# lan496/torch-m3gnet

Measured on AMD Instinct MI355X. Metric: atom-steps/sec (energy+forces) on 10k-atom PBC batch, 1/2/4/8 MI355X, higher is better.
Workload: dtype f32; 1 GPU; single 10000-atom fcc Cu PBC supercell per GPU (10x10x25 cells, a=3.61 A, jitter 0.025 A), r_cut 5 A / 3-body 4 A, default M3GNet (l_max=n_max=3, D=64, 3 blocks), energy+forces+stress; precision=fp32, atoms_per_gpu=10000, edges_per_gpu=420000, triplets_per_gpu=3060000

## Files before the change

### torch-m3gnet_amd/csrc/m3g_api.hip

```cpp
#include <climits>
#include <cmath>
#include <cstdarg>
#include <cstdio>
#include <cstdlib>
#include <cstring>
#include <utility>

#include "m3g_internal.h"

namespace m3g {

static thread_local char g_err[512] = "";
void set_error(const char* fmt, ...) {
  va_list ap;
  va_start(ap, fmt);
  vsnprintf(g_err, sizeof(g_err), fmt, ap);
  va_end(ap);
}

static void layout_mlp(MlpW& m, size_t& off) {
  auto take = [&](size_t n) { size_t r = off; off += (n + 63) / 64 * 64; return r; };
  m.w1a_t = take(kDP * 2 * kDP); m.w1b_t = take(kDP * 2 * kDP); m.w1c_t = take(kDP * 2 * kDP);
  m.b1 = take(2 * kDP);
  m.w2d_t = take(kDP * kDP); m.w2g_t = take(kDP * kDP);
// ... 277 lines not shown
  auto it = exp.find(key);
  if (it == exp.end()) { set_error("unknown parameter key '%s'", key); return M3G_ERR_VALUE; }
  if (it->second != numel) { set_error("parameter '%s': expected %lld values, got %lld", key, (long long)it->second, (long long)numel); return M3G_ERR_VALUE; }
  plan->params[key].assign(host_data, host_data + numel);
  plan->committed = false;
  return M3G_OK;
}

extern "C" int m3g_plan_set_const(m3g_plan* plan, const char* name, const float* host_data, int64_t numel) {
  if (!plan || !name || !host_data) { set_error("m3g_plan_set_const: null argument"); return M3G_ERR_VALUE; }
  auto exp = expected_consts(plan->cfg);
  auto it = exp.find(name);
  if (it == exp.end()) { set_error("unknown constant '%s'", name); return M3G_ERR_VALUE; }
  if (it->second != numel) { set_error("constant '%s': expected %lld values, got %lld", name, (long long)it->second, (long long)numel); return M3G_ERR_VALUE; }
  plan->cvals[name].assign(host_data, host_data + numel);
  plan->committed = false;
  return M3G_OK;
}

static int hook_stamps(m3g_plan* plan, int32_t* value) {
  if (*value && !plan->d_stamps) {
    M3G_HIP_CHECK(hipMalloc((void**)&plan->d_stamps, 256 * 16 * 12 * sizeof(unsigned long long)));
    M3G_HIP_CHECK(hipMemset(plan->d_stamps, 0, 256 * 16 * 12 * sizeof(unsigned long long)));
  } else if (!*value && plan->d_stamps) {
    (void)hipFree(plan->d_stamps);
    plan->d_stamps = nullptr;
  }
  *value = *value == 0 ? 0 : *value == 3 ? 3 : *value == 2 ? 2 : 1;
  return M3G_OK;
}
struct OptionRow {
  const char* name;
  int Options::*member;
  int lo, hi;
  const char* error;
  int (*hook)(m3g_plan*, int32_t* value);
};
#define M3G_HOOK(...) [](m3g_plan* plan, int32_t* value) -> int { __VA_ARGS__; return M3G_OK; }
static const OptionRow kOptions[] = {
    {"edge_kernel", &Options::edge_kernel, 0, 2, "edge_kernel must be 0 (VALU baseline), 1 (MFMA) or 2 (any-size path)",
     M3G_HOOK(if (plan->generic && *value != 2) { set_error("this model size only runs on the any-size path (edge_kernel = 2)"); return M3G_ERR_UNSUPPORTED; })},
    {"precision", &Options::precision, 0, 2,
     "precision must be 0 (fp32: exact fp32 MFMA products), 1 (bf16x3 split products) or 2 (f16x3: scaled fp16 split products)", nullptr},
    {"save_p1", &Options::save_p1, 0, 1, nullptr, nullptr},
    {"save_p2", &Options::save_p2, 0, 1, nullptr, nullptr},
    {"rev_kernel", &Options::rev_kernel, 0, 1, "rev_kernel must be 0 (node-MLP + edge-MLP kernel pair) or 1 (fused)", nullptr},
    {"small_tiles", &Options::small_tiles, 0, INT_MAX, "small_tiles must be >= 0", M3G_HOOK(plan->opt.small_tiles_fwd = *value)},
    {"small_tiles_fwd", &Options::small_tiles_fwd, 0, INT_MAX, "small_tiles_fwd must be >= 0", nullptr},
    {"dp1_by_dst", &Options::dp1_by_dst, 0, 1, nullptr, nullptr},
    {"split_node_tiles", &Options::split_node_tiles, 0, INT_MAX, "split_node_tiles must be >= 0", nullptr},
    {"species_tables", &Options::species_tables, 0, 1, nullptr, nullptr},
    {"fuse_node_tb", &Options::fuse_node_tb, 0, 1, nullptr, nullptr},
    {"debug_node_tb_polls", &Options::debug_node_tb_polls, INT_MIN, INT_MAX, nullptr, nullptr},
    {"split_tail", &Options::split_tail, 0, 2, "split_tail must be 0 (never), 1 (a single left-over tile) or 2 (one or two)", nullptr},
    {"small_launches", &Options::small_launches, 0, 1, nullptr, nullptr},
    {"graph_replay", &Options::graph_replay, 0, 1, nullptr, M3G_HOOK(if (!*value) drop_graphs(plan))},
    {"overlap", &Options::overlap, 0, 1, nullptr, nullptr},
    {"threebody_moments", &Options::tb_moments, 0, 1, nullptr, nullptr},
    {"legendre_backward", &Options::legendre_ref, 0, 1, "legendre_backward: 0 (exact derivative) or 1 (the reference's backward)", nullptr},
    {"readout_f16", &Options::readout_f16, 0, 1, nullptr, nullptr},
    {"stress_mode", &Options::stress_mode, 0, 1, "stress_mode must be 0 (reference: sum pos (x) F / V) or 1 (pair virial)", nullptr},
    {"debug_force_move", nullptr, INT_MIN, INT_MAX, nullptr, M3G_HOOK(plan->debug_force_move = *value != 0; plan->committed = false)},
    {"stamps", &Options::stamp_target, INT_MIN, INT_MAX, nullptr, hook_stamps},
};
#undef M3G_HOOK

extern "C" int m3g_plan_set_option(m3g_plan* plan, const char* name, int32_t value) {
  if (!plan || !name) { set_error("m3g_plan_set_option: null argument"); return M3G_ERR_VALUE; }
  for (const OptionRow& row : kOptions) {
    if (strcmp(name, row.name) != 0) continue;
    if (value < row.lo || value > row.hi) {
      if (row.error) { set_error("%s", row.error); return M3G_ERR_VALUE; }
      value = 1;
    }
    if (row.hook) { int rc = row.hook(plan, &value); if (rc) return rc; }
    if (row.member) plan->opt.*row.member = value;
    return M3G_OK;
  }
  set_error("unknown option '%s'", name);
  return M3G_ERR_VALUE;
}

extern "C" int m3g_debug_read_stamps(m3g_plan* plan, uint64_t* host_out ) {
  if (!plan || !host_out || !plan->d_stamps) { set_error("stamps not enabled"); return M3G_ERR_STATE; }
  M3G_HIP_CHECK(hipMemcpy(host_out, plan->d_stamps, 256 * 16 * 12 * sizeof(unsigned long long), hipMemcpyDeviceToHost));
  return M3G_OK;
}

extern "C" int m3g_plan_commit(m3g_plan* plan) {
  if (!plan) { set_error("m3g_plan_commit: null plan"); return M3G_ERR_VALUE; }
  drop_graphs(plan);
  const m3g_config& cfg = plan->cfg;
  for (auto& kv : expected_params(cfg))
    if (!plan->params.count(kv.first)) { set_error("parameter '%s' was never set", kv.first.c_str()); return M3G_ERR_STATE; }
  for (auto& kv : expected_consts(cfg))
    if (!plan->cvals.count(kv.first)) { set_error("constant '%s' was never set", kv.first.c_str()); return M3G_ERR_STATE; }
  const int D = cfg.embedding_dim, R = cfg.n_max, L = cfg.l_max, C = L * R, B = cfg.num_blocks;
  {
    int dev = 0;
    M3G_HIP_CHECK(hipGetDevice(&dev));
    if (plan->device >= 0 && (plan->device != dev || plan->debug_force_move)) {
      M3G_HIP_CHECK(hipSetDevice(plan->device));
      M3G_HIP_CHECK(hipDeviceSynchronize());
      if (plan->d_weights) { (void)hipFree(plan->d_weights); plan->d_weights = nullptr; }
      free_mfma_images(plan);
      generic_free(plan);
// ... 176 lines not shown

int Step::enqueue_optional_outputs() const {
  M3G_STAGE(ST_OUTPUTS);
  if (io->node_features) launch_copy_strided(w.x[c.B], kDP, io->node_features, c.D, c.D, t.N, s);
  if (io->edge_attr) {
    if (mfma) launch_soa_to_rows(w.e_blk[c.B], io->edge_attr, c.D, c.D, t.E, s);
    else launch_copy_strided(w.e, kDP, io->edge_attr, c.D, c.D, t.E, s);
  }
  if (io->edge_distances && t.E > 0) M3G_HIP_CHECK(hipMemcpyAsync(io->edge_distances, w.d, sizeof(float) * t.E, hipMemcpyDeviceToDevice, s));
  if (io->edge_weights) launch_copy_strided(w.h, kRP, io->edge_weights, c.R, c.R, t.E, s);
  if (io->triplet_angles) launch_triplet_angles(t, io->triplet_edge_index, w.u, io->triplet_angles, s);
  if (io->mid_edge_features)
    for (int b = 0; b < c.B; ++b)
      launch_copy_expand_rows(t.act_id, w.m[b], kCP, io->mid_edge_features + (size_t)b * t.E * c.C, c.C, c.C, t.E, s);
  return M3G_OK;
}

int Step::enqueue_reverse() const {
  float *dx_cur = w.dx, *dx_alt = w.dx2;
  bool dr_done = false;
  if (!mfma && c.B > 0 && t.E > 0) {
    M3G_HIP_CHECK(hipMemsetAsync(w.de, 0, sizeof(float) * t.E * kDP, s));
    M3G_HIP_CHECK(hipMemsetAsync(w.dh, 0, sizeof(float) * t.E * kRP, s));
  }
  for (int b = c.B - 1; b >= 0; --b) {
    const bool first = b == c.B - 1;
    switch (p.rev_edge) {
      case kRevSplit: { M3G_STAGE(ST_EDGE_REV_FUSED); launch_edge_rev_split(plan, p, c, t, w, b, dx_cur, first, s); } break;
      case kRevF32: { M3G_STAGE(ST_EDGE_REV_FUSED); launch_edge_rev_f32(plan, p, c, t, w, b, dx_cur, first, s); } break;
      case kRevFused: { M3G_STAGE(ST_EDGE_REV_FUSED); launch_edge_rev_fused(plan, c, t, w, b, dx_cur, first, s); } break;
      case kRevPair: {
        { M3G_STAGE(ST_EDGE_REV_NODE); launch_edge_rev_node_mlp(plan, p, c, t, w, b, dx_cur, s); }
        M3G_STAGE(ST_EDGE_REV);
        launch_edge_rev_edge_mlp(plan, p, c, t, w, b, dx_cur, first, s);
      } break;
      default: { M3G_STAGE(ST_EDGE_REV); launch_edge_block_reverse(c, W, wl.blk[b], t, w, b, dx_cur, s); }
    }
    bool node_done = false;
    if (p.tail[b] == kTailOverlap) {
      if (!ensure_side_stream(plan)) { set_error("overlap: could not create the internal stream"); return M3G_ERR_HIP; }
      M3G_HIP_CHECK(hipEventRecord(plan->ev_fork, s));
      M3G_HIP_CHECK(hipStreamWaitEvent(plan->side_stream, plan->ev_fork, 0));
      launch_threebody_reverse(p, c, t, w, w.v[b], first, plan->side_stream, plan->opt.legendre_ref);
      M3G_HIP_CHECK(hipEventRecord(plan->ev_join, plan->side_stream));
      launch_node_reverse(c, W, wl.blk[b], t, w, w.v[b], dx_cur, dx_alt, true, p.dp1, false, s);
      M3G_HIP_CHECK(hipStreamWaitEvent(s, plan->ev_join, 0));
      launch_node_reverse_v_term(c, W, wl.blk[b], t, w, w.v[b], dx_alt, s);
      node_done = true;
    } else if (p.tail[b] == kTailNodeTb) {
      node_done = launch_node_tb_reverse(c, W, wl.blk[b], t, w, w.v[b], first, dx_cur, dx_alt, p.dp1, b, s, p.tb_hints, plan->opt.debug_node_tb_polls);
    } else if (p.tail[b] == kTailFinalTb) {
      launch_threebody_reverse_final(c, t, w, w.v[b], first, w.dh_parts, c.B, s, p.tb_hints);
      dr_done = true;
    }
    if (!node_done && p.tail[b] != kTailFinalTb) {
      { M3G_STAGE(ST_THREEBODY_REV); launch_threebody_reverse(p, c, t, w, w.v[b], first, s, plan->opt.legendre_ref); }
      if (b > 0) {
        M3G_STAGE(ST_NODE_REV);
        launch_node_reverse(c, W, wl.blk[b], t, w, w.v[b], dx_cur, dx_alt, p.fused_rev, p.dp1, true, s, p.node_rev_small);
        node_done = true;
      }
    }
    if (node_done) std::swap(dx_cur, dx_alt);
  }
  {
    M3G_STAGE(ST_EMBED_REV);
    if (p.fused_rev) {  }
    else if (mfma) launch_embed_edges_reverse_soa(W + wl.adj, w.h, w.de_soa, w.dh_parts + (size_t)2 * c.B * t.E * kRP, t.E, s);
    else launch_embed_reverse(c, W, wl, t, w, s);
  }
  M3G_STAGE(ST_GEOM_REV);
  if (mfma) launch_geometry_reverse(c, t, w, w.dh_parts, p.fused_rev ? c.B : 2 * c.B + 1, io->forces, io->stresses, s, p.gather_virial, io->pos, io->lattice, dr_done);
  else launch_geometry_reverse(c, t, w, w.dh, 1, io->forces, io->stresses, s);
  if (p.stress == kStressPair) launch_stress_pair(t, w, io->lattice, io->stresses, s);
  else if (p.stress == kStressRef) launch_stress(c, t, io->pos, io->lattice, io->forces, io->stresses, s, p.energy_deferred ? ea : nullptr, st, io->total_energy);
  return M3G_OK;
}

static int enqueue_step(const m3g_plan* plan, const m3g_io* io, void* workspace, size_t workspace_bytes, hipStream_t s, RunMode mode) {
  const int64_t N = io->n_atoms, E = io->n_edges, T = io->n_triplets, S = io->n_structs;
  if (N < 0 || E < 0 || T < 0 || S < 0) { set_error("negative size"); return M3G_ERR_VALUE; }
  if (!io->total_energy || !io->topo || (N > 0 && (!io->pos || !io->atom_types)) || (S > 0 && !io->lattice) || (E > 0 && !io->edge_cell_shift)) {
    set_error("m3g_energy_forces: missing required pointer");
    return M3G_ERR_VALUE;
  }
  if (io->triplet_angles && T > 0 && !io->triplet_edge_index) { set_error("triplet_angles requires triplet_edge_index"); return M3G_ERR_VALUE; }
  const StepPath p = plan_step_path(plan, N, E, T, S, io->topo_hints, io->forces != nullptr, io->stresses != nullptr, mode.profile);
  if (p.pipeline == kPipeAnySize) return generic_energy_forces(plan, io, workspace, workspace_bytes, s);
  Step k{plan, io, p, p.pipeline == kPipeMfma, plan->consts, plan->wl, plan->d_weights, s, mode, topo_carve(N, E, T, S, const_cast<void*>(io->topo)),
         work_carve(plan->cfg.num_blocks, p, N, E, S, workspace)};
  if (!workspace || workspace_bytes < k.w.total_bytes) { set_error("workspace too small: %zu < %zu", workspace_bytes, k.w.total_bytes); return M3G_ERR_SIZE; }
  k.ea = io->scaled_atomic_energies ? io->scaled_atomic_energies : k.w.tail;
  k.st = io->scaled_total_energy ? io->scaled_total_energy : k.w.tail + N;
  { int rc = k.enqueue_forward(); if (rc) return rc; }
  { int rc = k.enqueue_optional_outputs(); if (rc) return rc; }
  if (io->forces) { int rc = k.enqueue_reverse(); if (rc) return rc; }
  else if (io->stresses) { set_error("stresses require forces"); return M3G_ERR_VALUE; }
  M3G_HIP_CHECK(hipGetLastError());
  return M3G_OK;
}

static int capture_step(const m3g_plan* plan, const m3g_io* io, void* workspace, size_t workspace_bytes, hipStream_t s, hipGraph_t* graph) {
  M3G_HIP_CHECK(hipStreamBeginCapture(s, hipStreamCaptureModeThreadLocal));
  const int rc = enqueue_step(plan, io, workspace, workspace_bytes, s, RunMode{false});
  const hipError_t e = hipStreamEndCapture(s, graph);
  if (rc != M3G_OK) { if (*graph) (void)hipGraphDestroy(*graph); return rc; }
// ... 127 lines not shown
```

### torch-m3gnet_amd/csrc/m3g_internal.h

```cpp
#pragma once
#include <hip/hip_runtime.h>

#include <cmath>
#include <cstddef>
#include <cstdint>
#include <map>
#include <string>
#include <vector>

#include "../../include/m3gnet_hip.h"
#include "m3g_step_path.h"

namespace m3g {

constexpr int kDP = 64;
constexpr int kLCap = 4;
constexpr int kRCap = 4;
constexpr int kRAnyCap = 10;
constexpr int kCP = 16;
constexpr int kRP = 4;

void set_error(const char* fmt, ...);
#define M3G_HIP_CHECK(expr)                                                               \
  do {                                                                                    \
// ... 319 lines not shown
void launch_stress(const Consts& c, const Topo& t, const float* pos, const float* lattice, const float* forces,
                   float* stresses, hipStream_t s, const float* ea = nullptr, float* scaled_total = nullptr, float* total = nullptr);
void launch_stress_pair(const Topo& t, const Work& w, const float* lattice, float* stresses, hipStream_t s);
void launch_force_gather(float length_scale, const Topo& t, const float* dr, float* forces, float* stresses, hipStream_t s);
size_t generic_workspace_bytes(const m3g_plan* plan, int64_t N, int64_t E, int64_t T, int64_t S);
int generic_commit(m3g_plan* plan);
void generic_free(m3g_plan* plan);
int generic_energy_forces(const m3g_plan* plan, const m3g_io* io, void* workspace, size_t workspace_bytes, hipStream_t s);
void generic_edge_featurizer(int n_max, double rc, const float* coeff, const float* em, const float* dm, int64_t E, const float* d, float* out,
                             hipStream_t s);
void launch_triplet_angles(const Topo& t, const int64_t* tei, const float* u, float* out, hipStream_t s);
void launch_distance_only(float length_scale, const Topo& t, const float* pos, const float* lattice,
                          const int32_t* shift, float* u, float* d, hipStream_t s);
void launch_edge_featurizer(const Consts& c, int64_t E, const float* d, float* out, int out_stride, hipStream_t s);
void launch_embed(const Consts& c, const float* W, const WeightLayout& wl, const Topo& t, const int64_t* types,
                  const Work& w, hipStream_t s);
void launch_embed_reverse(const Consts& c, const float* W, const WeightLayout& wl, const Topo& t, const Work& w,
                          hipStream_t s);
void launch_node_pre(const Consts& c, const float* W, const BlockW& bw, const Topo& t, const Work& w, const float* x_prev, float* x,
                     float* v, float* TA, float* TB, hipStream_t s);
void launch_node_pre_mfma(const m3g_plan* plan, bool split, const Consts& c, const Topo& t, const Work& w, int b, const float* x_prev, float* x,
                          float* v, float* TA, float* TB, const int64_t* types, const float* emb, hipStream_t s);
void launch_geometry_node_pre(const m3g_plan* plan, const Consts& c, const Topo& t, const Work& w, const float* pos, const float* lattice,
                              const int32_t* shift, const int64_t* types, const float* emb, hipStream_t s);
void launch_species_expand(const m3g_plan* plan, const Consts& c, const Topo& t, const Work& w, const int64_t* types, hipStream_t s);
void launch_geometry_species(const m3g_plan* plan, const Consts& c, const Topo& t, const Work& w, const float* pos, const float* lattice,
                             const int32_t* shift, const int64_t* types, hipStream_t s);
int build_species_tables(m3g_plan* plan);
void launch_energy_sums(const Consts& c, const Topo& t, const float* scaled_atomic, float* scaled_total, float* total, hipStream_t s);
void launch_readout_mfma(const m3g_plan* plan, const StepPath& p, const Consts& c, const WeightLayout& wl, const Topo& t, const int64_t* types,
                         const float* x_prev, float* x, const Work& w, float* scaled_atomic, float* scaled_total, float* total,
                         bool want_grad, hipStream_t s);
void launch_node_reverse(const Consts& c, const float* W, const BlockW& bw, const Topo& t, const Work& w,
                         const float* v, const float* dx_new, float* dx_out, bool row_sums_in_seg, int dp1_packed, bool with_v_term,
                         hipStream_t s, bool small = false);
void launch_node_reverse_v_term(const Consts& c, const float* W, const BlockW& bw, const Topo& t, const Work& w, const float* v,
                                float* dx_out, hipStream_t s);
void launch_readout(const Consts& c, const float* W, const WeightLayout& wl, const Topo& t, const int64_t* types,
                    const float* x_prev, float* x, const Work& w, float* scaled_atomic, float* scaled_total, float* total,
                    bool want_grad, hipStream_t s);
void launch_gather_rows(const float* table, int64_t n, int width, int table_stride, int table_rows, bool transposed,
                        const int64_t* idx, float* out, hipStream_t s);
void launch_copy_expand_rows(const int32_t* row_id, const float* in, int in_stride, float* out, int out_stride, int width, int64_t n,
                             hipStream_t s);
void launch_copy_strided(const float* in, int in_stride, float* out, int out_stride, int width, int64_t rows,
                         hipStream_t s);
void launch_threebody(const StepPath& p, const Consts& c, const Topo& t, const Work& w, const float* v, float* m, hipStream_t s);
void launch_threebody_reverse(const StepPath& p, const Consts& c, const Topo& t, const Work& w, const float* v, bool first, hipStream_t s,
                              bool ref_legendre = false);
void launch_threebody_reverse_final(const Consts& c, const Topo& t, const Work& w, const float* v, bool first, const float* dh, int dh_parts,
                                    hipStream_t s, int topo_hints);
bool launch_node_tb_reverse(const Consts& c, const float* W, const BlockW& bw, const Topo& t, const Work& w, const float* v, bool first,
                            const float* dx_new, float* dx_out, int dp1_packed, int block, hipStream_t s, int topo_hints, int debug_polls = 0);
int pack_mfma_images(m3g_plan* plan);
void free_mfma_images(m3g_plan* plan);
void launch_edge_block_mfma(const m3g_plan* plan, const StepPath& p, const Consts& c, const Topo& t, const Work& w, int b, hipStream_t s,
                            bool e_out_read = true);
void launch_edge_rev_node_mlp(const m3g_plan* plan, const StepPath& p, const Consts& c, const Topo& t, const Work& w, int b, const float* dx_new,
                              hipStream_t s);
void launch_edge_rev_edge_mlp(const m3g_plan* plan, const StepPath& p, const Consts& c, const Topo& t, const Work& w, int b, const float* dx_new,
                              bool de_is_zero, hipStream_t s);
void launch_edge_rev_fused(const m3g_plan* plan, const Consts& c, const Topo& t, const Work& w, int b, const float* dx_new,
                           bool de_is_zero, hipStream_t s);
void launch_edge_rev_f32(const m3g_plan* plan, const StepPath& p, const Consts& c, const Topo& t, const Work& w, int b, const float* dx_new,
                         bool de_is_zero, hipStream_t s);
void launch_edge_fwd_split(const m3g_plan* plan, const StepPath& p, const Consts& c, const Topo& t, const Work& w, int b, hipStream_t s);
void launch_edge_rev_split(const m3g_plan* plan, const StepPath& p, const Consts& c, const Topo& t, const Work& w, int b, const float* dx_new, bool de_is_zero,
                           hipStream_t s);
void launch_embed_edges_soa(const Consts& c, const float* adj_t, const float* h, float* soa, int64_t E, hipStream_t s);
void launch_embed_edges_reverse_soa(const float* adj, const float* h, const float* de_soa, float* dh_slice, int64_t E, hipStream_t s);
void launch_embed_nodes_only(const Consts& c, const float* W, const WeightLayout& wl, const Topo& t, const int64_t* types,
                             const Work& w, hipStream_t s);
void launch_rows_to_soa(const float* rows, float* soa, int64_t E, hipStream_t s);
void launch_soa_to_rows(const float* soa, float* rows, int row_stride, int width, int64_t E, hipStream_t s);
void launch_edge_block(const Consts& c, const float* W, const BlockW& bw, const Topo& t, const Work& w, int b,
                       const float* x_old, float* x_new, hipStream_t s);
void launch_edge_block_reverse(const Consts& c, const float* W, const BlockW& bw, const Topo& t, const Work& w, int b,
                               const float* dx_new, hipStream_t s);

}
```

### torch-m3gnet_amd/csrc/m3g_node.hip

```cpp
#include "m3g_internal.h"
#include "m3g_device.h"
#include "m3g_mfma_common.h"
#include "m3g_node_rev.h"

namespace m3g {


__global__ void __launch_bounds__(256) k_embed_nodes(int64_t N, int num_types, const int64_t* __restrict__ types,
                                                     const float* __restrict__ emb, float* __restrict__ x) {
  int64_t idx = blockIdx.x * (int64_t)blockDim.x + threadIdx.x;
  if (idx >= N * kDP) return;
  int64_t a = idx / kDP;
  int o = (int)(idx % kDP);
  bool bad;
  x[idx] = emb[species_index(types[a], num_types, bad) * kDP + o];
}

__global__ void __launch_bounds__(256) k_embed_edges(int R, int64_t E, const float* __restrict__ adj_t, const float* __restrict__ h,
                                                     float* __restrict__ e0) {
  int64_t idx = blockIdx.x * (int64_t)blockDim.x + threadIdx.x;
  if (idx >= E * kDP) return;
  int64_t e = idx / kDP;
  int o = (int)(idx % kDP);
  float p = 0.f;
// ... 48 lines not shown
    xs[nb][k] = a < N ? node_feature(ns, x, a, k) : 0.f;
  }
  __syncthreads();
  int o = tid;
  const MlpW& mw = o < 2 * kDP ? bw.e : bw.n;
  int oo = o < 2 * kDP ? o : o - 2 * kDP;
  float accA[kNodesPerBlock], accB[kNodesPerBlock];
  float bias = W[mw.b1 + oo];
#pragma unroll
  for (int nb = 0; nb < kNodesPerBlock; ++nb) { accA[nb] = bias; accB[nb] = 0.f; }
  const float* wa = W + mw.w1a_t + oo;
  const float* wb = W + mw.w1b_t + oo;
#pragma unroll 8
  for (int k = 0; k < kDP; ++k) {
    float a = wa[k * 2 * kDP], b = wb[k * 2 * kDP];
#pragma unroll
    for (int nb = 0; nb < kNodesPerBlock; ++nb) {
      float xv = xs[nb][k];
      accA[nb] += a * xv;
      accB[nb] += b * xv;
    }
  }
#pragma unroll
  for (int nb = 0; nb < kNodesPerBlock; ++nb) {
    int64_t a = n0 + nb;
    if (a < N) { TA[a * 4 * kDP + o] = accA[nb]; TB[a * 4 * kDP + o] = accB[nb]; }
  }
  static_assert(kNodesPerBlock * kCP <= 256, "one thread per (atom, c)");
  if (tid < kNodesPerBlock * kCP) {
    int nb = tid / kCP, c = tid % kCP;
    int64_t a = n0 + nb;
    if (a < N) {
      float p = W[bw.tb_b1 + c];
      for (int k = 0; k < kDP; ++k) p += W[bw.tb_w1_t + k * kCP + c] * xs[nb][k];
      v[a * kCP + c] = c < C ? sigmoid_f(p) : 0.f;
    }
  }
}

__global__ void __launch_bounds__(256) k_node_reverse(NodeRevArgs a) {
  node_reverse_body<false>(a, blockIdx.x, [] { return false; });
}
__global__ void __launch_bounds__(256) k_node_reverse_small(NodeRevArgs a) {
  node_reverse_body<false, true>(a, blockIdx.x, [] { return false; });
}

__global__ void __launch_bounds__(256) k_node_reverse_v_term(int C, int64_t N, const float* __restrict__ W, size_t tb_w1,
                                                             const int32_t* __restrict__ in_ptr, const int32_t* __restrict__ in_edge,
                                                             const float* __restrict__ dgq, const float* __restrict__ v,
                                                             float* __restrict__ dx_out, const int2* __restrict__ in_pair) {
  __shared__ float tv[16][kCP];
  const int g = threadIdx.x >> 4, cq = threadIdx.x & 15;
  const int64_t i = (int64_t)blockIdx.x * 16 + g;
  float dv = 0.f;
  if (i < N) {
    int k = in_ptr[i];
    const int k1 = in_ptr[i + 1];
    auto row = [&](int kk) { const int ar = in_pair[kk].y; return ar >= 0 ? dgq[(int64_t)ar * kCP + cq] : 0.f; };
    for (; k + 3 < k1; k += 4) dv += (row(k) + row(k + 1)) + (row(k + 2) + row(k + 3));
    for (; k < k1; ++k) dv += row(k);
    (void)in_edge;
    const float vv = v[i * kCP + cq];
    dv = cq < C ? dv * vv * (1.f - vv) : 0.f;
  }
  tv[g][cq] = dv;
  __syncthreads();
  for (int idx = threadIdx.x; idx < 16 * kDP; idx += 256) {
    const int nb = idx >> 6, k = idx & 63;
    const int64_t a = (int64_t)blockIdx.x * 16 + nb;
    if (a >= N) continue;
    float acc = 0.f;
    for (int cc = 0; cc < C; ++cc) acc += tv[nb][cc] * W[tb_w1 + cc * kDP + k];
    dx_out[a * kDP + k] += acc;
  }
}

constexpr int kRA = 4;
__global__ void __launch_bounds__(256) k_readout(Consts c, int64_t N, const float* __restrict__ W, ReadoutW rw,
                                                 size_t elemental_off, const int64_t* __restrict__ types,
                                                 const float* __restrict__ x, NodeSums ns, float* __restrict__ scaled_atomic,
                                                 float* __restrict__ dx, float* __restrict__ scaled_total, int64_t S, const int32_t* topo_flags) {
  __shared__ float bufA[4][kRA][kDP], bufB[4][kRA][kDP];
  if (blockIdx.x == 0) for (int64_t i = threadIdx.x; i < S; i += blockDim.x) scaled_total[i] = 0.f;
  const int wv = threadIdx.x >> 6, o = threadIdx.x & 63;
  const int64_t a0 = ((int64_t)blockIdx.x * 4 + wv) * kRA;
#pragma unroll
  for (int j = 0; j < kRA; ++j) bufA[wv][j][o] = a0 + j < N ? node_feature(ns, x, a0 + j, o) : 0.f;
  __syncthreads();
  float pd1[kRA], pg1[kRA], pd2[kRA], pg2[kRA];
  {
    const float bd = W[rw.b1d + o], bg = W[rw.b1g + o];
#pragma unroll
    for (int j = 0; j < kRA; ++j) { pd1[j] = bd; pg1[j] = bg; }
    for (int k = 0; k < kDP; ++k) {
      const float wd = W[rw.w1d_t + k * kDP + o], wg = W[rw.w1g_t + k * kDP + o];
#pragma unroll
      for (int j = 0; j < kRA; ++j) { const float xv = bufA[wv][j][k]; pd1[j] += wd * xv; pg1[j] += wg * xv; }
    }
  }
#pragma unroll
  for (int j = 0; j < kRA; ++j) { bufA[wv][j][o] = silu_f(pd1[j]); bufB[wv][j][o] = silu_f(pg1[j]); }
  __syncthreads();
  {
    const float bd = W[rw.b2d + o], bg = W[rw.b2g + o];
#pragma unroll
    for (int j = 0; j < kRA; ++j) { pd2[j] = bd; pg2[j] = bg; }
    for (int k = 0; k < kDP; ++k) {
      const float wd = W[rw.w2d_t + k * kDP + o], wg = W[rw.w2g_t + k * kDP + o];
#pragma unroll
      for (int j = 0; j < kRA; ++j) { pd2[j] += wd * bufA[wv][j][k]; pg2[j] += wg * bufB[wv][j][k]; }
    }
  }
  const float w3d = W[rw.w3d + o], w3g = W[rw.w3g + o];
  float od[kRA], og[kRA], sg[kRA];
#pragma unroll
  for (int j = 0; j < kRA; ++j) {
    od[j] = w3d * silu_f(pd2[j]);
    og[j] = w3g * silu_f(pg2[j]);
    for (int off = 32; off > 0; off >>= 1) { od[j] += __shfl_xor(od[j], off); og[j] += __shfl_xor(og[j], off); }
    od[j] += W[rw.b3];
    og[j] += W[rw.b3 + 1];
    sg[j] = sigmoid_f(og[j]);
    if (a0 + j < N && o == 0) {
      bool bad;
      const int64_t ty = species_index(types[a0 + j], c.num_types, bad);
      scaled_atomic[a0 + j] = bad ? __builtin_nanf("") : W[elemental_off + ty] / c.energy_scale + od[j] * sg[j];
// ... 142 lines not shown
```

### torch-m3gnet_amd/csrc/m3g_step_path.h

```cpp
#pragma once
#include <cstdint>

#include "../../include/m3gnet_hip.h"

namespace m3g {

constexpr int kMaxBlocks = 8;
constexpr int kPrecF32 = 0;
constexpr int kPrecBf16x3 = 1;
constexpr int kPrecF16x3 = 2;
constexpr int kNumPrec = 3;

constexpr int kSyncWords = 16;
constexpr int kSyncForceTail = 0, kSyncReadout = 1, kSyncNodeRev = 2;
constexpr int64_t kForceTailMaxStructs = 8;
constexpr int64_t kFusedSumsMaxAtoms = 1024;
constexpr int64_t kNodeTbFusedMaxAtoms = 128;

constexpr int32_t topo_hints_word(int32_t bad, int32_t rows, int32_t atoms) {
  return (bad == 0 && rows > 0) ? (M3G_TOPO_TB_COMPLETE | ((rows & 0xff) << 8) | ((atoms & 0xff) << 16)) : 0;
}
constexpr int topo_hints_rows(int hints) { return (hints >> 8) & 0xff; }
constexpr int topo_hints_atoms(int hints) { return (hints >> 16) & 0xff; }

struct Options {
  int precision = kPrecF32;
  int save_p1 = 1;
  int save_p2 = 1;
  int small_tiles_fwd = 3072;
  int small_tiles = 1536;
  int dp1_by_dst = 0;
  int split_node_tiles = 128;
  int species_tables = 1;
  int fuse_node_tb = 1;
  int debug_node_tb_polls = 0;
  int split_tail = 1;
  int small_launches = 1;
  int rev_kernel = 1;
  int readout_f16 = 0;
  int legendre_ref = 0;
  int tb_moments = 1;
  int stress_mode = 0;
  int edge_kernel = 1;
  int stamp_target = 0;
  int overlap = 0;
  int graph_replay = 0;
};
static_assert(sizeof(Options) == 21 * sizeof(int), "Options: twenty-one ints, no padding (its bytes are compared as a key)");

enum { kDp1F32 = 0, kDp1Packed = 1, kDp1Fixed = 2, kDp1F32ByDst = 3  };

enum Pipeline { kPipeValu = 0, kPipeMfma = 1, kPipeAnySize = 2 };
enum RevEdge { kRevValu = 0, kRevPair, kRevFused, kRevF32, kRevSplit };
enum Readout { kReadoutValu = 0, kReadoutSplit, kReadoutF32, kReadoutF16 };
enum RevTail {
  kTailSeparate = 0,
  kTailOverlap,
  kTailNodeTb,
  kTailFinalTb,
};
enum Block0Tables {
  kBlock0Kernel = 0,
  kBlock0ExpandBesideGeom,
  kBlock0ExpandAlone,
};
enum StressKernel { kStressNone = 0, kStressInGather , kStressPair, kStressRef };

struct ModelDims { int L, R, C, B; };

struct StepPath {
  int pipeline = kPipeMfma;
  bool fused_rev = false;
  int saved_acts = 0;
  int fwd_save = 0;
  int dp1 = kDp1F32;
  bool dp1_by_dst = false;
  int tb_hints = 0;
  bool moments = false;
  bool long_lists = false;
  bool geom_with_node_pre = false;
  int block0 = kBlock0Kernel;
  bool node_split = false;
  bool fwd_split = false;
  int rev_edge = kRevValu;
  int split_tail = 0;
  int readout = kReadoutValu;
  bool readout_sums = false;
  bool energy_deferred = false;
  int tail[kMaxBlocks] = {};
  bool node_rev_small = false;
  bool gather_virial = false;
  int stress = kStressNone;
};

inline StepPath resolve_step_path(const Options& o, const ModelDims& m, int64_t N, int64_t E, int64_t T, int64_t S, int topo_hints,
                                  bool want_forces, bool want_stresses, bool profile) {
  StepPath p;
  p.pipeline = o.edge_kernel;
  if (o.edge_kernel == 2) return p;
  const bool mfma = o.edge_kernel == 1, f32 = o.precision == kPrecF32, stamps = o.stamp_target != 0;
  const bool saves_p1 = mfma && f32 && o.save_p1 != 0;
  const bool saves_p2 = saves_p1 && o.rev_kernel == 1 && o.save_p2 != 0;
  p.saved_acts = saves_p2 ? 2 : saves_p1 ? 1 : 0;
  p.fwd_save = want_forces ? p.saved_acts : 0;
  p.fused_rev = mfma && o.rev_kernel == 1 && (!f32 || saves_p1);
  p.dp1_by_dst = o.dp1_by_dst && p.fused_rev && f32;
  p.dp1 = !p.fused_rev ? kDp1F32 : p.dp1_by_dst ? kDp1F32ByDst : o.precision == kPrecBf16x3 ? kDp1Packed : o.precision == kPrecF16x3 ? kDp1Fixed : kDp1F32;

  p.tb_hints = o.tb_moments && !o.legendre_ref ? topo_hints : 0;
  p.moments = (p.tb_hints & M3G_TOPO_TB_COMPLETE) && m.L >= 1 && m.L <= 3 && m.R >= 1 && m.R <= 4 && topo_hints_rows(p.tb_hints) > 0 &&
              topo_hints_atoms(p.tb_hints) > 0;
  p.long_lists = T > 24 * E;
  const bool tb_mom = p.moments && E != 0 && T != 0;

  const int64_t etiles = (E + 15) / 16, ntiles = (N + 15) / 16;
  const bool small_nodes = o.small_launches && ntiles <= o.split_node_tiles;
  const bool few = N <= kFusedSumsMaxAtoms && S > 0 && S <= kForceTailMaxStructs;
  if (mfma) {
    p.node_split = f32 && small_nodes;
    p.geom_with_node_pre = !profile && p.node_split && m.B != 0 && E != 0 && N != 0;
    if (o.species_tables && m.B != 0 && N != 0) p.block0 = !profile && E != 0 ? kBlock0ExpandBesideGeom : kBlock0ExpandAlone;
    p.fwd_split = etiles > 0 && etiles <= o.small_tiles_fwd && f32 && p.fwd_save != 1 && !stamps;
    p.rev_edge = !p.fused_rev ? kRevPair : !f32 ? kRevFused : (etiles > 0 && etiles <= o.small_tiles && saves_p2 && !stamps) ? kRevSplit : kRevF32;
    p.split_tail = o.split_tail;
    const bool f16_readout = o.precision == kPrecF16x3 && o.readout_f16;
    p.readout = f16_readout ? kReadoutF16 : small_nodes ? kReadoutSplit : kReadoutF32;
    p.readout_sums = o.small_launches && N > 0 && few;
    p.energy_deferred = o.small_launches && want_forces && want_stresses && o.stress_mode == 0 && !profile && !p.readout_sums && N > 0;
  }
  if (!want_forces) return p;
  for (int b = 0; b < m.B && b < kMaxBlocks; ++b) {
    if (b > 0 && p.fused_rev && o.overlap && !profile) p.tail[b] = kTailOverlap;
    else if (b > 0 && p.fused_rev && o.fuse_node_tb && !profile && N <= kNodeTbFusedMaxAtoms && N != 0 && tb_mom && kSyncNodeRev + b < kSyncWords)
      p.tail[b] = kTailNodeTb;
    else if (b == 0 && p.fused_rev && o.small_launches && !profile && tb_mom) p.tail[b] = kTailFinalTb;
  }
  p.node_rev_small = o.small_launches && N <= kFusedSumsMaxAtoms;
  p.gather_virial = mfma && o.small_launches && o.stress_mode == 0 && want_stresses && N > 0 && few;
  p.stress = !want_stresses ? kStressNone : p.gather_virial ? kStressInGather : o.stress_mode == 1 ? kStressPair : kStressRef;
  return p;
}

}
```

### torch-m3gnet_amd/csrc/m3g_threebody.hip

```cpp
#include <algorithm>
#include <map>
#include <mutex>
#include <utility>

#include "m3g_internal.h"
#include "m3g_node_rev.h"
#include "m3g_geometry_body.h"

namespace m3g {


template <int C>
__device__ __forceinline__ void load_row(const float* __restrict__ row, float* out) {
#pragma unroll
  for (int k = 0; k < C; k += 4) {
    const float4 t = *(const float4*)(row + k);
    out[k] = t.x;
    if (k + 1 < C) out[k + 1] = t.y;
    if (k + 2 < C) out[k + 2] = t.z;
    if (k + 3 < C) out[k + 3] = t.w;
  }
}

struct TbArgs {
// ... 431 lines not shown
          const MomEval eg = mom_eval<L>(s_mom + (at * R + nn) * NM, ux, uy, uz, s2, g0, g1, g2);
          const MomEval eh = mom_eval<L>(s_mom + ((cap_atoms + at) * R + nn) * NM, ux, uy, uz, s2, d0, d1, d2);
          dfc += dmv[nn] * (c.ynorm[0] * eg.S0);
          dg[nn] = c.ynorm[0] * eh.S0;
          if constexpr (L >= 2) {
            dfc += dmv[R + nn] * (c.ynorm[1] * eg.S1);
            dg[R + nn] = c.ynorm[1] * eh.S1;
            ax += c.ynorm[1] * (d1 * eg.V1x + g1 * eh.V1x);
            ay += c.ynorm[1] * (d1 * eg.V1y + g1 * eh.V1y);
            az += c.ynorm[1] * (d1 * eg.V1z + g1 * eh.V1z);
          }
          if constexpr (L >= 3) {
            dfc += dmv[2 * R + nn] * (c.ynorm[2] * eg.S2);
            dg[2 * R + nn] = c.ynorm[2] * eh.S2;
            ax += c.ynorm[2] * (d2 * eg.V2x + g2 * eh.V2x);
            ay += c.ynorm[2] * (d2 * eg.V2y + g2 * eh.V2y);
            az += c.ynorm[2] * (d2 * eg.V2z + g2 * eh.V2z);
          }
        }
        float ddv = 0.f, val[kCP];
#pragma unroll
        for (int k = 0; k < kCP; ++k) {
          val[k] = 0.f;
          if (k < C) {
            const int kc = k < C ? k : 0;
            ddv += dg[kc] * vv[kc] * qpv[kc];
            val[k] = dg[kc] * qv[kc];
          }
        }
#pragma unroll
        for (int k = 0; k < kCP; k += 4) *(float4*)(a.dgq + (int64_t)r * kCP + k) = float4{val[k], val[k + 1], val[k + 2], val[k + 3]};
        a.dd[r] = (dd0 + fcp * dfc) + ddv;
        a.du[(int64_t)r * 3] = du0 + ax;
        a.du[(int64_t)r * 3 + 1] = du1 + ay;
        a.du[(int64_t)r * 3 + 2] = du2 + az;
        if constexpr (FINAL) {
          float rx, ry, rz;
          edge_dr(a.geom, e, rx, ry, rz);
          a.dr[e * 3] = rx; a.dr[e * 3 + 1] = ry; a.dr[e * 3 + 2] = rz;
        }
      }
    }
    __syncthreads();
  }
  if constexpr (FINAL) {
    for (int64_t e = (int64_t)vblock * THREADS + threadIdx.x; e < a.geom.E; e += (int64_t)vgrid * THREADS) {
      if (a.geom.act_id[e] >= 0) continue;
      float rx, ry, rz;
      edge_dr(a.geom, e, rx, ry, rz);
      a.dr[e * 3] = rx; a.dr[e * 3 + 1] = ry; a.dr[e * 3 + 2] = rz;
    }
  }
}
constexpr int kTbMomThreads = 128;
template <int L, int R, bool REV>
__global__ void __launch_bounds__(kTbMomThreads) k_threebody_moments(Consts c, TbMomArgs a, int cap_rows, int cap_atoms) {
  extern __shared__ __attribute__((aligned(16))) float lds_mom[];
  tb_moments_body<L, R, REV, kTbMomThreads>(c, a, cap_rows, cap_atoms, (int)blockIdx.x, (int)gridDim.x, lds_mom);
}
template <int L, int R>
__global__ void __launch_bounds__(kTbMomThreads) k_threebody_moments_final(Consts c, TbMomArgs a, int cap_rows, int cap_atoms) {
  extern __shared__ __attribute__((aligned(16))) float lds_mom[];
  tb_moments_body<L, R, true, kTbMomThreads, true>(c, a, cap_rows, cap_atoms, (int)blockIdx.x, (int)gridDim.x, lds_mom);
}

struct NodeTbArgs {
  int n_tb;
  int32_t* done;
  int max_polls;
  int wait_extra;
};
template <int L, int R>
__global__ void __launch_bounds__(256) k_node_tb_reverse(Consts c, TbMomArgs ta, int cap_rows, int cap_atoms, NodeRevArgs na, NodeTbArgs f) {
  extern __shared__ __attribute__((aligned(16))) float lds_mom[];
  if ((int)blockIdx.x < f.n_tb) {
    tb_moments_body<L, R, true, 256>(c, ta, cap_rows, cap_atoms, (int)blockIdx.x, f.n_tb, lds_mom);
    __builtin_amdgcn_fence(__ATOMIC_RELEASE, "agent");
    __syncthreads();
    if (threadIdx.x == 0) __hip_atomic_fetch_add(f.done, 1, __ATOMIC_RELAXED, __HIP_MEMORY_SCOPE_AGENT);
    return;
  }
  node_reverse_body<true, true>(na, (int64_t)blockIdx.x - f.n_tb, [&] {
    int never_came = 0;
    if ((threadIdx.x & 63) == 0) {
      int spins = 0;
      while (__hip_atomic_load(f.done, __ATOMIC_RELAXED, __HIP_MEMORY_SCOPE_AGENT) < f.n_tb + f.wait_extra) {
        __builtin_amdgcn_s_sleep(16);
        if (++spins > f.max_polls) { atomicOr(ta.flags + 8, M3G_TOPO_ERR_SYNC); never_came = 1; break; }
      }
    }
    __builtin_amdgcn_fence(__ATOMIC_ACQUIRE, "agent");
    return __builtin_amdgcn_readfirstlane(never_came) != 0;
  });
}

constexpr int kTbGridCap = 2048;
static inline dim3 grid_rows(int64_t n) {
  const int64_t blocks = (n + kTbRows - 1) / kTbRows;
  return dim3((unsigned)(blocks < kTbGridCap ? blocks : kTbGridCap));
}
template <class A>
static A tb_args(const Topo& t, const Work& w, const float* v) {
  A a{};
  a.act_list = t.act_list; a.act_dst = t.act_dst; a.tb_win = t.tb_win; a.n_act = t.n_act;
  a.u = w.u; a.fc3 = w.fc3; a.q = w.q; a.v = v;
  return a;
}
template <class A>
static void tb_reverse_fields(A& a, const Work& w, bool first) {
  a.fc3p = w.fc3p; a.qp = w.qp; a.dm = w.dm;
  a.dd = w.dd; a.du = w.du; a.dgq = w.dg; a.first = first ? 1 : 0;
}
static TbMomArgs tb_mom_args(const Topo& t, const Work& w, const float* v, int topo_hints, float* m, bool first) {
  TbMomArgs a = tb_args<TbMomArgs>(t, w, v);
  a.blocks = (int)tb_win_blocks(t.E);
  a.src = t.src; a.arow_ptr = t.arow_ptr; a.tb_fast = t.tb_fast; a.flags = t.flags; a.hints = topo_hints;
// ... 19 lines not shown
}
struct TbShortLists { static constexpr int LIST = kTbListShort, CAP = kTbCapShort, LPR = kTbLprShort; };
struct TbLongLists { static constexpr int LIST = kTbListLong, CAP = kTbCap, LPR = kTbLprLong; };
#define M3G_TB_LIST_LAUNCH(KERNEL, V, c, a, s) \
  M3G_DISPATCH_LR((c).L, (c).R, hipLaunchKernelGGL((KERNEL<L, R, V::LIST, V::CAP, V::LPR>), grid_rows((a).E), dim3(kTbRows * V::LPR), 0, s, c, a))
#define M3G_TB_LIST_DISPATCH(KERNEL, long_lists, c, a, s) \
  if (long_lists) { M3G_TB_LIST_LAUNCH(KERNEL, TbLongLists, c, a, s); } else { M3G_TB_LIST_LAUNCH(KERNEL, TbShortLists, c, a, s); }

void launch_threebody(const StepPath& p, const Consts& c, const Topo& t, const Work& w, const float* v, float* m, hipStream_t s) {
  if (t.E == 0) return;
  if (t.T == 0) return;
  if (p.moments) return launch_moments<false>(c, tb_mom_args(t, w, v, p.tb_hints, m, false), t.E, s);
  TbArgs a = tb_args<TbArgs>(t, w, v);
  a.E = t.E; a.t_ptr = t.t1_ptr; a.t_other = t.t1_e2c; a.t_bytes = t.t1_b; a.m = m;
  M3G_TB_LIST_DISPATCH(k_threebody_fwd, p.long_lists, c, a, s);
}

template <int L, int R>
static bool node_tb_launch(const Consts& c, const TbMomArgs& a, const NodeRevArgs& na, int n_tb, int n_node, int32_t* done, int debug_polls,
                           hipStream_t s) {
  const MomDims d = mom_dims<L, R, true>(a.hints);
  static std::mutex mu;
  static std::map<std::pair<int, size_t>, int> resident;
  int dev = 0, cap = 0;
  if (hipGetDevice(&dev) != hipSuccess) return false;
  {
    std::lock_guard<std::mutex> lock(mu);
    auto it = resident.find(std::make_pair(dev, d.lds));
    if (it == resident.end()) {
      int per_cu = 0, cus = 0;
      if (hipOccupancyMaxActiveBlocksPerMultiprocessor(&per_cu, k_node_tb_reverse<L, R>, 256, d.lds) != hipSuccess ||
          hipDeviceGetAttribute(&cus, hipDeviceAttributeMultiprocessorCount, dev) != hipSuccess)
        per_cu = cus = 0;
      it = resident.emplace(std::make_pair(dev, d.lds), per_cu * cus).first;
    }
    cap = it->second;
  }
  if (n_tb + n_node > cap) return false;
  const NodeTbArgs f{n_tb, done, debug_polls > 0 ? debug_polls : debug_polls < 0 ? -debug_polls : 1 << 22, debug_polls < 0 ? 1 : 0};
  hipLaunchKernelGGL((k_node_tb_reverse<L, R>), dim3((unsigned)(n_tb + n_node)), dim3(256), d.lds, s, c, a, d.rows, d.atoms, na, f);
  return true;
}

bool launch_node_tb_reverse(const Consts& c, const float* W, const BlockW& bw, const Topo& t, const Work& w, const float* v, bool first,
                            const float* dx_new, float* dx_out, int dp1_packed, int block, hipStream_t s, int topo_hints, int debug_polls) {
  const TbMomArgs a = tb_mom_args(t, w, v, topo_hints, nullptr, first);
  const NodeRevArgs na = node_rev_args(c, W, bw, t, w, v, dx_new, dx_out, true, dp1_packed, true);
  const int n_tb = (int)std::min<unsigned>(grid_rows(t.E).x, 128u), n_node = (int)((t.N + kNodesRev - 1) / kNodesRev);
  bool launched = false;
  M3G_DISPATCH_LR3(c.L, c.R, launched = (node_tb_launch<L, R>(c, a, na, n_tb, n_node, w.sync + kSyncNodeRev + block, debug_polls, s)));
  return launched;
}

void launch_threebody_reverse_final(const Consts& c, const Topo& t, const Work& w, const float* v, bool first, const float* dh, int dh_parts,
                                    hipStream_t s, int topo_hints) {
  TbMomArgs a = tb_mom_args(t, w, v, topo_hints, nullptr, first);
  a.geom = GeomRev{t.E, w.u, w.d, w.hp, dh, dh_parts, w.dd, w.du, t.act_id};
  a.dr = w.dr;
  launch_moments<true, true>(c, a, t.E, s);
}

void launch_threebody_reverse(const StepPath& p, const Consts& c, const Topo& t, const Work& w, const float* v, bool first, hipStream_t s,
                              bool ref_legendre) {
  if (t.E == 0) return;
  if (t.T == 0) return;
  if (p.moments) return launch_moments<true>(c, tb_mom_args(t, w, v, p.tb_hints, nullptr, first), t.E, s);
  TbRevArgs a = tb_args<TbRevArgs>(t, w, v);
  tb_reverse_fields(a, w, first);
  a.E = t.E; a.ref_legendre = ref_legendre ? 1 : 0;
  a.t1_ptr = t.t1_ptr; a.t1_other = t.t1_e2c; a.t1_bytes = t.t1_b;
  a.t2_ptr = t.t2_ptr; a.t2_other = t.t2_e1c; a.t2_bytes = t.t2_b;
  M3G_TB_LIST_DISPATCH(k_threebody_rev, p.long_lists, c, a, s);
}

}
```

Before: 4.238 million atom-steps/s.

## Add opt-in role-split kernel co-running three-body and node reverse; restructure v-term kernel

Adds a kernel whose blocks take either a three-body-moment role or a node-reverse role, interleaved by a configurable split. The aim is to co-schedule the two reverse stages in one launch for large systems, but it sits behind a new option that is off by default. It also rewrites the node-reverse v-term kernel. Weights and existing outputs are preloaded into registers, neighbour rows are gathered in batches of 64 via shuffles, and each output is written once rather than loaded inside the inner loop. The large unrolled gather array may raise register pressure.

```diff
diff --git a/torch-m3gnet_amd/csrc/m3g_api.hip b/torch-m3gnet_amd/csrc/m3g_api.hip
--- a/torch-m3gnet_amd/csrc/m3g_api.hip
+++ b/torch-m3gnet_amd/csrc/m3g_api.hip
@@ -353,6 +353,7 @@
     {"species_tables", &Options::species_tables, 0, 1, nullptr, nullptr},
     {"fuse_node_tb", &Options::fuse_node_tb, 0, 1, nullptr, nullptr},
     {"debug_node_tb_polls", &Options::debug_node_tb_polls, INT_MIN, INT_MAX, nullptr, nullptr},
+    {"tail_roles", &Options::tail_roles, 0, INT_MAX, "tail_roles must be >= 0", nullptr},
     {"split_tail", &Options::split_tail, 0, 2, "split_tail must be 0 (never), 1 (a single left-over tile) or 2 (one or two)", nullptr},
     {"small_launches", &Options::small_launches, 0, 1, nullptr, nullptr},
     {"graph_replay", &Options::graph_replay, 0, 1, nullptr, M3G_HOOK(if (!*value) drop_graphs(plan))},
@@ -635,6 +636,10 @@
     } else if (p.tail[b] == kTailFinalTb) {
       launch_threebody_reverse_final(c, t, w, w.v[b], first, w.dh_parts, c.B, s, p.tb_hints);
       dr_done = true;
+    } else if (p.tail_roles[b]) {
+      launch_node_tb_roles(c, W, wl.blk[b], t, w, w.v[b], first, dx_cur, dx_alt, p.dp1, p.node_rev_small, s, p.tb_hints, plan->opt.tail_roles);
+      launch_node_reverse_v_term(c, W, wl.blk[b], t, w, w.v[b], dx_alt, s);
+      node_done = true;
     }
     if (!node_done && p.tail[b] != kTailFinalTb) {
       { M3G_STAGE(ST_THREEBODY_REV); launch_threebody_reverse(p, c, t, w, w.v[b], first, s, plan->opt.legendre_ref); }
diff --git a/torch-m3gnet_amd/csrc/m3g_internal.h b/torch-m3gnet_amd/csrc/m3g_internal.h
--- a/torch-m3gnet_amd/csrc/m3g_internal.h
+++ b/torch-m3gnet_amd/csrc/m3g_internal.h
@@ -395,6 +395,8 @@
                                     hipStream_t s, int topo_hints);
 bool launch_node_tb_reverse(const Consts& c, const float* W, const BlockW& bw, const Topo& t, const Work& w, const float* v, bool first,
                             const float* dx_new, float* dx_out, int dp1_packed, int block, hipStream_t s, int topo_hints, int debug_polls = 0);
+void launch_node_tb_roles(const Consts& c, const float* W, const BlockW& bw, const Topo& t, const Work& w, const float* v, bool first,
+                          const float* dx_new, float* dx_out, int dp1_packed, bool small, hipStream_t s, int topo_hints, int split);
 int pack_mfma_images(m3g_plan* plan);
 void free_mfma_images(m3g_plan* plan);
 void launch_edge_block_mfma(const m3g_plan* plan, const StepPath& p, const Consts& c, const Topo& t, const Work& w, int b, hipStream_t s,
diff --git a/torch-m3gnet_amd/csrc/m3g_node.hip b/torch-m3gnet_amd/csrc/m3g_node.hip
--- a/torch-m3gnet_amd/csrc/m3g_node.hip
+++ b/torch-m3gnet_amd/csrc/m3g_node.hip
@@ -124,26 +124,47 @@
   __shared__ float tv[16][kCP];
   const int g = threadIdx.x >> 4, cq = threadIdx.x & 15;
   const int64_t i = (int64_t)blockIdx.x * 16 + g;
+  const int k = threadIdx.x & 63, nb0 = threadIdx.x >> 6;
+  float acc[4], wk[kCP];
+#pragma unroll
+  for (int m = 0; m < 4; ++m) {
+    const int64_t a = (int64_t)blockIdx.x * 16 + nb0 + 4 * m;
+    acc[m] = a < N ? dx_out[a * kDP + k] : 0.f;
+  }
+#pragma unroll
+  for (int cc = 0; cc < kCP; ++cc) wk[cc] = cc < C ? W[tb_w1 + cc * kDP + k] : 0.f;
   float dv = 0.f;
   if (i < N) {
-    int k = in_ptr[i];
-    const int k1 = in_ptr[i + 1];
-    auto row = [&](int kk) { const int ar = in_pair[kk].y; return ar >= 0 ? dgq[(int64_t)ar * kCP + cq] : 0.f; };
-    for (; k + 3 < k1; k += 4) dv += (row(k) + row(k + 1)) + (row(k + 2) + row(k + 3));
-    for (; k < k1; ++k) dv += row(k);
+    const int k0 = in_ptr[i], k1 = in_ptr[i + 1];
+    const float vv = v[i * kCP + cq];
+    for (int kb = k0; kb < k1; kb += 64) {
+      int mine[4];
+#pragma unroll
+      for (int q = 0; q < 4; ++q) mine[q] = kb + 16 * q + cq < k1 ? in_pair[kb + 16 * q + cq].y : -1;
+      float gr[64];
+#pragma unroll
+      for (int j = 0; j < 64; ++j) {
+        const int ar = __shfl(mine[j >> 4], j & 15, 16);
+        gr[j] = ar >= 0 ? dgq[(int64_t)ar * kCP + cq] : 0.f;
+      }
+#pragma unroll
+      for (int j = 0; j < 64; j += 4) dv += (gr[j] + gr[j + 1]) + (gr[j + 2] + gr[j + 3]);
+    }
     (void)in_edge;
-    const float vv = v[i * kCP + cq];
     dv = cq < C ? dv * vv * (1.f - vv) : 0.f;
   }
   tv[g][cq] = dv;
   __syncthreads();
-  for (int idx = threadIdx.x; idx < 16 * kDP; idx += 256) {
-    const int nb = idx >> 6, k = idx & 63;
+#pragma unroll
+  for (int m = 0; m < 4; ++m) {
+    const int nb = nb0 + 4 * m;
     const int64_t a = (int64_t)blockIdx.x * 16 + nb;
     if (a >= N) continue;
-    float acc = 0.f;
-    for (int cc = 0; cc < C; ++cc) acc += tv[nb][cc] * W[tb_w1 + cc * kDP + k];
-    dx_out[a * kDP + k] += acc;
+    float r = acc[m];
+#pragma unroll
+    for (int cc = 0; cc < kCP; ++cc)
+      if (cc < C) r += tv[nb][cc] * wk[cc];
+    dx_out[a * kDP + k] = r;
   }
 }
 
diff --git a/torch-m3gnet_amd/csrc/m3g_step_path.h b/torch-m3gnet_amd/csrc/m3g_step_path.h
--- a/torch-m3gnet_amd/csrc/m3g_step_path.h
+++ b/torch-m3gnet_amd/csrc/m3g_step_path.h
@@ -34,6 +34,7 @@
   int species_tables = 1;
   int fuse_node_tb = 1;
   int debug_node_tb_polls = 0;
+  int tail_roles = 0;
   int split_tail = 1;
   int small_launches = 1;
   int rev_kernel = 1;
@@ -46,7 +47,7 @@
   int overlap = 0;
   int graph_replay = 0;
 };
-static_assert(sizeof(Options) == 21 * sizeof(int), "Options: twenty-one ints, no padding (its bytes are compared as a key)");
+static_assert(sizeof(Options) == 22 * sizeof(int), "Options: twenty-two ints, no padding (its bytes are compared as a key)");
 
 enum { kDp1F32 = 0, kDp1Packed = 1, kDp1Fixed = 2, kDp1F32ByDst = 3  };
 
@@ -88,6 +89,7 @@
   bool readout_sums = false;
   bool energy_deferred = false;
   int tail[kMaxBlocks] = {};
+  bool tail_roles[kMaxBlocks] = {};
   bool node_rev_small = false;
   bool gather_virial = false;
   int stress = kStressNone;
@@ -134,6 +136,7 @@
     else if (b > 0 && p.fused_rev && o.fuse_node_tb && !profile && N <= kNodeTbFusedMaxAtoms && N != 0 && tb_mom && kSyncNodeRev + b < kSyncWords)
       p.tail[b] = kTailNodeTb;
     else if (b == 0 && p.fused_rev && o.small_launches && !profile && tb_mom) p.tail[b] = kTailFinalTb;
+    p.tail_roles[b] = b > 0 && p.fused_rev && o.tail_roles && !profile && !o.overlap && N > kNodeTbFusedMaxAtoms && tb_mom && p.tail[b] == kTailSeparate;
   }
   p.node_rev_small = o.small_launches && N <= kFusedSumsMaxAtoms;
   p.gather_virial = mfma && o.small_launches && o.stress_mode == 0 && want_stresses && N > 0 && few;
diff --git a/torch-m3gnet_amd/csrc/m3g_threebody.hip b/torch-m3gnet_amd/csrc/m3g_threebody.hip
--- a/torch-m3gnet_amd/csrc/m3g_threebody.hip
+++ b/torch-m3gnet_amd/csrc/m3g_threebody.hip
@@ -507,6 +507,20 @@
     }
   }
 }
+struct RoleSplit { int n_a, every, start; };
+struct Role { bool a; int index; };
+__device__ __forceinline__ Role role_of(int b, const RoleSplit& f) {
+  if (b < f.start) return Role{false, b};
+  const int period = f.every + 1, rel = b - f.start, q = rel / period;
+  if (rel % period == 0 && q < f.n_a) return Role{true, q};
+  const int before = (rel + period - 1) / period;
+  return Role{false, b - (before < f.n_a ? before : f.n_a)};
+}
+static RoleSplit role_split(int n_a, int n_b, int every, int start = 0) {
+  start = start < 0 ? 0 : start > n_b ? n_b : start;
+  if (n_a > 0 && every > (n_b - start) / n_a) every = (n_b - start) / n_a;
+  return RoleSplit{n_a, every < 0 ? 0 : every, start};
+}
 constexpr int kTbMomThreads = 128;
 template <int L, int R, bool REV>
 __global__ void __launch_bounds__(kTbMomThreads) k_threebody_moments(Consts c, TbMomArgs a, int cap_rows, int cap_atoms) {
@@ -517,6 +531,14 @@
 __global__ void __launch_bounds__(kTbMomThreads) k_threebody_moments_final(Consts c, TbMomArgs a, int cap_rows, int cap_atoms) {
   extern __shared__ __attribute__((aligned(16))) float lds_mom[];
   tb_moments_body<L, R, true, kTbMomThreads, true>(c, a, cap_rows, cap_atoms, (int)blockIdx.x, (int)gridDim.x, lds_mom);
+}
+
+template <int L, int R, bool SMALL>
+__global__ void __launch_bounds__(256) k_node_tb_roles(Consts c, TbMomArgs ta, int cap_rows, int cap_atoms, NodeRevArgs na, RoleSplit f) {
+  extern __shared__ __attribute__((aligned(16))) float lds_mom[];
+  const Role role = role_of((int)blockIdx.x, f);
+  if (role.a) return tb_moments_body<L, R, true, 256>(c, ta, cap_rows, cap_atoms, role.index, f.n_a, lds_mom);
+  node_reverse_body<false, SMALL>(na, role.index, [] { return false; });
 }
 
 struct NodeTbArgs {
@@ -642,6 +664,26 @@
   return launched;
 }
 
+constexpr int kTailRolesTb = 512, kTailRolesEvery = 1;
+template <int L, int R, bool SMALL>
+static void node_tb_roles_launch(const Consts& c, const TbMomArgs& a, const NodeRevArgs& na, const RoleSplit& f, int n_node, hipStream_t s) {
+  const MomDims d = mom_dims<L, R, true>(a.hints);
+  hipLaunchKernelGGL((k_node_tb_roles<L, R, SMALL>), dim3((unsigned)(f.n_a + n_node)), dim3(256), d.lds, s, c, a, d.rows, d.atoms, na, f);
+}
+void launch_node_tb_roles(const Consts& c, const float* W, const BlockW& bw, const Topo& t, const Work& w, const float* v, bool first,
+                          const float* dx_new, float* dx_out, int dp1_packed, bool small, hipStream_t s, int topo_hints, int split) {
+  const TbMomArgs a = tb_mom_args(t, w, v, topo_hints, nullptr, first);
+  const NodeRevArgs na = node_rev_args(c, W, bw, t, w, v, dx_new, dx_out, true, dp1_packed, false);
+  const int row_blocks = (int)grid_rows(t.E).x, n_node = (int)((t.N + kNodesRev - 1) / kNodesRev);
+  const bool sweep = split > 1;
+  const int want_tb = sweep ? (split & 0xffff) : kTailRolesTb, want_every = sweep ? (split >> 16) & 0xff : kTailRolesEvery;
+  const int start = sweep ? ((split >> 25) & 0x3f) * 64 : 0;
+  const int n_tb = want_tb > 0 && want_tb < row_blocks ? want_tb : row_blocks;
+  const RoleSplit f = role_split(n_tb, n_node, want_every, start);
+  if (small) { M3G_DISPATCH_LR3(c.L, c.R, (node_tb_roles_launch<L, R, true>(c, a, na, f, n_node, s))); }
+  else { M3G_DISPATCH_LR3(c.L, c.R, (node_tb_roles_launch<L, R, false>(c, a, na, f, n_node, s))); }
+}
+
 void launch_threebody_reverse_final(const Consts& c, const Topo& t, const Work& w, const float* v, bool first, const float* dh, int dh_parts,
                                     hipStream_t s, int topo_hints) {
   TbMomArgs a = tb_mom_args(t, w, v, topo_hints, nullptr, first);
```

Result: no change. 4.237 million atom-steps/s (-0.0%).
